# lmxyy/sige

Hardware: AMD Instinct MI355X
Metric: DDPM-256 U-Net sparse (SIGE) forwards/s (higher is better)
Workload: dtype f32; 1 GPU; DDPM 256x256 church U-Net (ch128, mult 1-1-2-2-4-4, 113.7M params, random init), 1.2% square edit, one edited image per GPU, hipGraph replay, NHWC activations, in-place scatter ...; batch_per_gpu=1, resolution=256, parallelism=dp1

## Files before the change

include/sige_hip.h:

```cpp
#ifndef SIGE_HIP_H
#define SIGE_HIP_H

#include <stddef.h>
#include <stdint.h>

#ifdef __cplusplus
extern "C" {
#endif

#define SIGE_HIP_VERSION 309

enum {
    SIGE_HIP_OK = 0,
    SIGE_HIP_EINVAL = -1,
    SIGE_HIP_EUNSUPPORTED = -2,
    SIGE_HIP_ELAUNCH = -3,
    SIGE_HIP_ENODEVICE = -4
};

enum { SIGE_HIP_ACT_IDENTITY = 0, SIGE_HIP_ACT_SWISH = 1,
       SIGE_HIP_ACT_RELU = 2, SIGE_HIP_ACT_LEAKY = 3 , SIGE_HIP_ACT_TANH = 4 };

enum {
    SIGE_HIP_TUNE_CONV_TILE_MT = 0,
// ... 63 lines not shown
                             const int32_t *active_indices, int N, int32_t *map, void *stream);

int sige_hip_scatter_gather_f32(const float *x, const float *y, int B, int C, int H, int W,
                                int Rx, int Sx, int bH, int bW,
                                const int32_t *active_indices, int N, const int32_t *scatter_map,
                                const float *scale, int scaleB, int scaleC, int scaleH, int scaleW,
                                const float *shift, int shiftB, int shiftC, int shiftH, int shiftW,
                                int activation, int activation_first, float *out, void *stream);

int sige_hip_difference_mask_u8(const float *a, const float *b, int C, int H, int W,
                                int64_t strideC, int64_t strideH, int64_t strideW, float eps,
                                uint8_t *out, void *stream);
int sige_hip_dilate_mask_u8(const uint8_t *mask, int H, int W, int dilationH, int dilationW,
                            uint8_t *out, void *stream);
int sige_hip_mask_pyramid_levels(int H, int W, int min_h, int min_w, int *hs, int *ws, int capacity);
int sige_hip_mask_pyramid_u8(const uint8_t *mask, int H, int W, int min_h, int min_w,
                             int dilationH, int dilationW, float threshold, float eps,
                             float *scratch, size_t scratch_floats, uint8_t *out, void *stream);

int sige_hip_reduce_mask_capacity(int H, int W, int strideH, int strideW, int padH, int padW);
int sige_hip_reduce_mask_i32(const uint8_t *mask, int H, int W, int bH, int bW,
                             int strideH, int strideW, int padH, int padW,
                             int32_t *indices, int capacity, int32_t *count, void *stream);

size_t sige_hip_block_conv_packed_size(int Cout, int Cin, int kH, int kW, int R, int S,
                                       int strideH, int strideW, int groups);
int sige_hip_block_conv_pack_f32(const float *w, int Cout, int Cin, int kH, int kW,
                                 float *packed, void *stream);
int sige_hip_block_conv_f32(const float *x, int T, int Cin, int R, int S,
                            const float *packed, const float *bias, int Cout, int kH, int kW,
                            int strideH, int strideW, float *out, void *stream);
int sige_hip_block_conv_direct_f32(const float *x, int T, int Cin, int R, int S,
                                   const float *w, const float *bias, int Cout, int kH, int kW,
                                   int strideH, int strideW, int dilationH, int dilationW, int groups,
                                   float *out, void *stream);
int sige_hip_spade_modulate_nhwc_f32(
        const float *x_full, const float *x_tiles, const int32_t *map_x, int Nx, int Rx, int Sx,
        const float *scale, int scaleB, int scaleC, const float *shift, int shiftB, int shiftC,
        const float *gb_tiles, const float *gb_full, const int32_t *map_g, int Ng, int Rg, int Sg,
        int B, int C, int H, int W, int bH, int bW, const int32_t *active_indices, int N,
        int leaky, float slope, float *out, void *stream);

size_t sige_hip_block_conv_packed_size_f16c(int Cout, int Cin, int kH, int kW, int R, int S,
                                            int strideH, int strideW, int groups);
int sige_hip_block_conv_pack_f16c(const float *w, int Cout, int Cin, int kH, int kW,
                                  float *packed, void *stream);
// ... 416 lines not shown
```

sige_amd/csrc/mask_pipeline.hip:

```cpp
#include "common.hpp"

namespace sige {

constexpr int kMPThreads = 1024;

__global__ void difference_mask_kernel(const float *__restrict__ a, const float *__restrict__ b, int C, long HW,
                                       long strideC, long stridePix, float eps, uint8_t *__restrict__ out) {
    for (long p = (long)blockIdx.x * blockDim.x + threadIdx.x; p < HW; p += (long)gridDim.x * blockDim.x) {
        bool any = false;
        for (int c = 0; c < C; ++c) {
            const long o = c * strideC + p * stridePix;
            any |= fabsf(a[o] - b[o]) > eps;
        }
        out[p] = any ? 1 : 0;
    }
}

__device__ __forceinline__ uint8_t dilated(const uint8_t *__restrict__ m, int W, int h, int w, int dH, int dW, int lo, int hi) {
    if (m[(size_t)h * W + w]) return 1;
    for (int i = 1; i <= dH; ++i) {
        if (h - i >= lo && m[(size_t)(h - i) * W + w]) return 1;
        if (h + i < hi && m[(size_t)(h + i) * W + w]) return 1;
    }
    for (int i = 1; i <= dW; ++i) {
// ... 57 lines not shown
        for (long p = tid; p < n2; p += kMPThreads) {
            const int i = (int)(p / w2), j = (int)(p % w2);
            float fy = sy * ((float)i + 0.5f) - 0.5f;
            if (fy < 0.f) fy = 0.f;
            const int y0 = (int)fy, y1 = y0 + (y0 < h - 1 ? 1 : 0);
            const float ly = fy - (float)y0, hy = 1.f - ly;
            float fx = sx * ((float)j + 0.5f) - 0.5f;
            if (fx < 0.f) fx = 0.f;
            const int x0 = (int)fx, x1 = x0 + (x0 < w - 1 ? 1 : 0);
            const float lx = fx - (float)x0, hx = 1.f - lx;
            auto at = [&](int y, int x) -> float {
                const size_t q = (size_t)y * w + x;
                return cur ? cur[q] : (mask[q] ? 1.0f : 0.0f);
            };
            nxt[p] = hy * (hx * at(y0, x0) + lx * at(y0, x1)) + ly * (hx * at(y1, x0) + lx * at(y1, x1));
        }
        __syncthreads();
        cur = nxt;
        nxt = (nxt == level_a) ? level_b : level_a;
        h = h2; w = w2;
    }
}

}

using namespace sige;

extern "C" int sige_hip_difference_mask_u8(const float *a, const float *b, int C, int H, int W,
                                           int64_t strideC, int64_t strideH, int64_t strideW, float eps,
                                           uint8_t *out, void *stream) {
    SIGE_PLAN_HOOK(sige_hip_difference_mask_u8, a, b, C, H, W, strideC, strideH, strideW, eps, out, stream);
    if (C <= 0 || H <= 0 || W <= 0) return SIGE_HIP_EINVAL;
    if (!a || !b || !out) return SIGE_HIP_EINVAL;
    if (strideH != (int64_t)W * strideW) return SIGE_HIP_EUNSUPPORTED;
    const long HW = (long)H * W;
    const int blocks = (int)((HW + 255) / 256 < 2048 ? (HW + 255) / 256 : 2048);
    difference_mask_kernel<<<blocks, 256, 0, as_stream(stream)>>>(a, b, C, HW, strideC, strideW, eps, out);
    return launch_status();
}

extern "C" int sige_hip_dilate_mask_u8(const uint8_t *mask, int H, int W, int dilationH, int dilationW,
                                       uint8_t *out, void *stream) {
    SIGE_PLAN_HOOK(sige_hip_dilate_mask_u8, mask, H, W, dilationH, dilationW, out, stream);
    if (H <= 0 || W <= 0 || dilationH < 0 || dilationW < 0) return SIGE_HIP_EINVAL;
    if (!mask || !out || mask == out) return SIGE_HIP_EINVAL;
    const long n = (long)H * W;
    const int blocks = (int)((n + 255) / 256 < 2048 ? (n + 255) / 256 : 2048);
    const int sh = stacked_shift(H);
    if (sh < 0) return SIGE_HIP_EUNSUPPORTED;
// ... 38 lines not shown
```

sige_amd/hip.py:

```python
import ctypes
import os
import threading
from typing import Optional, Tuple

import torch

_PKG = os.path.dirname(os.path.abspath(__file__))
LIB_PATH = os.environ.get("SIGE_HIP_LIB", os.path.join(_PKG, "lib", "libsige_hip.so"))

ACT = {"identity": 0, "swish": 1}
ACT_EXT = {"identity": 0, "relu": 2, "leaky": 3, "tanh": 4}

_c_int, _c_vp, _c_sz = ctypes.c_int, ctypes.c_void_p, ctypes.c_size_t
_lib = None

_BC = [_c_vp, _c_int, _c_int, _c_int, _c_int]

_SIGNATURES = {
    "sige_hip_version": (_c_int, []),
    "sige_hip_error_string": (ctypes.c_char_p, [_c_int]),
    "sige_hip_device_arch": (ctypes.c_char_p, []),
    "sige_hip_launch_count": (ctypes.c_int64, []),
    "sige_hip_last_launch_device": (_c_int, []),
    "sige_hip_preload": (_c_int, []),
    "sige_hip_gather_f32": (_c_int, [_c_vp] + [_c_int] * 6 + [_c_vp, _c_int] + _BC + _BC + [_c_int, _c_int, _c_vp, _c_vp]),
    "sige_hip_scatter_f32": (_c_int, [_c_vp, _c_vp] + [_c_int] * 10 + [_c_vp, _c_int] + _BC + [_c_vp, _c_vp]),
    "sige_hip_scatter_with_block_residual_f32": (
        _c_int, [_c_vp] * 4 + [_c_int] * 12 + [_c_vp, _c_int, _c_vp, _c_int, _c_vp, _c_vp]),
    "sige_hip_tile_table_i32": (_c_int, [_c_vp] + [_c_int] * 9 + [_c_vp, _c_vp]),
    "sige_hip_scatter_fused_f32": (_c_int, [_c_vp, _c_vp] + [_c_int] * 6 + [_c_vp, _c_int, _c_int, _c_int] + _BC + [_c_vp, _c_vp]),
    "sige_hip_scatter_with_block_residual_fused_f32": (
        _c_int, [_c_vp] * 4 + [_c_int] * 8 + [_c_vp, _c_int, _c_int, _c_int] * 2 + [_c_vp, _c_vp]),
    "sige_hip_scatter_map_i32": (_c_int, [_c_int] * 10 + [_c_vp, _c_int, _c_vp, _c_vp]),
    "sige_hip_scatter_gather_f32": (
        _c_int, [_c_vp, _c_vp] + [_c_int] * 8 + [_c_vp, _c_int, _c_vp] + _BC + _BC + [_c_int, _c_int, _c_vp, _c_vp]),
    "sige_hip_difference_mask_u8": (_c_int, [_c_vp, _c_vp] + [_c_int] * 3 + [ctypes.c_int64] * 3 + [ctypes.c_float, _c_vp, _c_vp]),
    "sige_hip_dilate_mask_u8": (_c_int, [_c_vp] + [_c_int] * 4 + [_c_vp, _c_vp]),
    "sige_hip_mask_pyramid_levels": (_c_int, [_c_int] * 4 + [_c_vp, _c_vp, _c_int]),
    "sige_hip_mask_pyramid_u8": (_c_int, [_c_vp] + [_c_int] * 6 + [ctypes.c_float] * 2 + [_c_vp, _c_sz, _c_vp, _c_vp]),
    "sige_hip_reduce_mask_capacity": (_c_int, [_c_int] * 6),
    "sige_hip_reduce_mask_i32": (_c_int, [_c_vp] + [_c_int] * 8 + [_c_vp, _c_int, _c_vp, _c_vp]),
    "sige_hip_block_conv_packed_size": (_c_sz, [_c_int] * 9),
    "sige_hip_block_conv_packed_size_f16c": (_c_sz, [_c_int] * 9),
    "sige_hip_block_conv_pack_f16c": (_c_int, [_c_vp] + [_c_int] * 4 + [_c_vp, _c_vp]),
    "sige_hip_block_conv_pack_f32": (_c_int, [_c_vp] + [_c_int] * 4 + [_c_vp, _c_vp]),
    "sige_hip_block_conv_f32": (_c_int, [_c_vp] + [_c_int] * 4 + [_c_vp, _c_vp] + [_c_int] * 5 + [_c_vp, _c_vp]),
    "sige_hip_gather_conv_f32": (
        _c_int, [_c_vp] + [_c_int] * 6 + [_c_vp, _c_int] + _BC + _BC + [_c_int, _c_vp, _c_vp] + [_c_int] * 5 + [_c_vp, _c_vp]),
    "sige_hip_scatter_gather_conv_f32": (
        _c_int, [_c_vp, _c_vp] + [_c_int] * 8 + [_c_vp, _c_int, _c_vp] + _BC + _BC + [_c_int, _c_vp, _c_vp]
        + [_c_int] * 5 + [_c_vp, _c_vp]),
    "sige_hip_gather_conv_nchw_f32": (
        _c_int, [_c_vp, _c_vp] + [_c_int] * 7 + [_c_vp, _c_int] + [_c_vp, _c_int, _c_int] * 2 + [_c_int, _c_vp, _c_vp]
        + [_c_int] * 7 + [_c_vp, _c_int, _c_int, _c_vp, _c_vp]),
    "sige_hip_group_norm_affine_workspace": (_c_sz, [_c_int] * 5),
    "sige_hip_group_norm_affine_f32": (_c_int, [_c_vp] + [_c_int] * 5 + [ctypes.c_float] + [_c_vp] * 6),
    "sige_hip_block_conv_direct_f32": (_c_int, [_c_vp] + [_c_int] * 4 + [_c_vp, _c_vp] + [_c_int] * 8 + [_c_vp, _c_vp]),
    "sige_hip_conv_pair_begin": (_c_int, []),
    "sige_hip_conv_pair_end": (_c_int, []),
    "sige_hip_conv_pairs_fused": (ctypes.c_int64, []),
    "sige_hip_attention_workspace": (_c_sz, [_c_int] * 3),
    "sige_hip_attention_f32": (_c_int, [_c_vp, _c_int, _c_int, _c_int, ctypes.c_float, _c_vp, _c_vp, _c_vp]),
    "sige_hip_copy_f32": (_c_int, [_c_vp, _c_vp, _c_sz, _c_vp]),
    "sige_hip_block_conv_nhwc_f32": (_c_int, [_c_vp] + [_c_int] * 4 + [_c_vp, _c_vp] + [_c_int] * 5 + [_c_vp, _c_vp]),
# ... 517 lines not shown
        table1.data_ptr(), table1.shape[0], table1.shape[1], n1, out.data_ptr(), _stream(y0)),
        "scatter_with_block_residual_fused")
    return out


def reduce_mask(mask: torch.Tensor, block_size, stride, padding) -> torch.Tensor:
    if mask.dim() != 2 or not mask.is_cuda:
        raise RuntimeError("sige_amd.hip.reduce_mask: expected a 2-D CUDA mask")
    if plan_recorder() is not None:
        return reduce_mask_batch([(mask, block_size, stride, padding)])[0]
    m = mask if mask.dtype in (torch.bool, torch.uint8) else (mask != 0)
    m = m.contiguous()
    H, W = m.shape
    cap = lib().sige_hip_reduce_mask_capacity(H, W, stride[0], stride[1], padding[0], padding[1])
    buf = torch.empty((cap + 1, 2), dtype=torch.int32, device=m.device)
    count = buf[cap]
    _check(lib().sige_hip_reduce_mask_i32(m.data_ptr(), H, W, block_size[0], block_size[1], stride[0], stride[1],
                                          padding[0], padding[1], buf.data_ptr(), cap, count.data_ptr(),
                                          _stream(m)), "reduce_mask")
    n = int(count[0].item())
    return buf[:n].clone()


def reduce_mask_batch(requests) -> list:
    if not requests:
        return []
    dev = requests[0][0].device
    counts = torch.empty(len(requests), dtype=torch.int32, device=dev)
    bufs = []
    for i, (mask, block, stride, padding) in enumerate(requests):
        if mask.dim() != 2 or not mask.is_cuda or mask.device != dev:
            raise RuntimeError("sige_amd.hip.reduce_mask_batch: expected 2-D masks on one GPU")
        m = mask if mask.dtype in (torch.bool, torch.uint8) else (mask != 0)
        m = m.contiguous()
        H, W = m.shape
        cap = lib().sige_hip_reduce_mask_capacity(H, W, stride[0], stride[1], padding[0], padding[1])
        buf = torch.empty((max(cap, 1), 2), dtype=torch.int32, device=dev)
        _check(lib().sige_hip_reduce_mask_i32(m.data_ptr(), H, W, block[0], block[1], stride[0], stride[1],
                                              padding[0], padding[1], buf.data_ptr(), cap,
                                              counts.data_ptr() + 4 * i, _stream(m)), "reduce_mask")
        bufs.append((buf, m))
    rec = plan_recorder()
    if rec is not None:
        first = rec.new_slots(len(requests))
        _check(lib().sige_hip_plan_record_readback(rec.handle, counts.data_ptr(), first, len(requests)), "plan_record_readback")
        ns = counts.cpu().tolist()
        out = []
        for i, ((buf, m), n) in enumerate(zip(bufs, ns)):
            rec.bind_index_list(buf, first + i, n)
            rec.keep.extend((buf, m))
            out.append(buf[:n])
        rec.keep.append(counts)
        return out
    ns = counts.cpu().tolist()
    return [buf[:n].clone() for (buf, _), n in zip(bufs, ns)]


def difference_mask(tensor1: torch.Tensor, tensor2: torch.Tensor, eps: float) -> torch.Tensor:
    if tensor1.shape != tensor2.shape:
        raise RuntimeError("difference_mask: shapes differ")
    a, b = tensor1, tensor2
    if a.dim() == 4:
        assert a.shape[0] == 1
        a, b = a[0], b[0]
    if a.dim() == 2:
        a, b = a[None], b[None]
    if a.dim() != 3:
        raise NotImplementedError("Unknown mask dimension [%d]!!!" % tensor1.dim())
    if not (a.is_cuda and b.is_cuda and a.dtype == b.dtype == torch.float32):
        raise NotImplementedError("difference_mask: fp32 GPU tensors")
    if a.stride() != b.stride() or a.stride(1) != a.shape[2] * a.stride(2):
        a, b = a.contiguous(), b.contiguous()
    C, H, W = a.shape
    out = torch.empty((H, W), dtype=torch.uint8, device=a.device)
    _check(lib().sige_hip_difference_mask_u8(a.data_ptr(), b.data_ptr(), C, H, W, a.stride(0), a.stride(1), a.stride(2),
                                             float(eps), out.data_ptr(), _stream(a)), "difference_mask")
    return out.view(torch.bool)

# ... 1289 lines not shown
```

sige_amd/nn/base.py:

```python
from typing import Dict, List, Optional, Tuple

import torch
from torch import nn
from torch.nn import functional as F

from .. import runtime as _runtime
from . import deferred

MODES = ("full", "sparse", "profile")


class _RuntimeTable(dict):

    def __init__(self, function_name: str):
        super().__init__()
        self.function_name = function_name

    def __missing__(self, device_type: str):
        fn = _runtime.resolve(device_type, self.function_name)
        if fn is not None:
            self[device_type] = fn
        return fn


# ... 183 lines not shown

    def _sige_modules(self):
        return (m for m in self.modules() if isinstance(m, SIGEModule))

    def set_masks(self, masks: Dict[Tuple[int, int], torch.Tensor]):
        self.timestamp += 1
        cache = {}
        self._prebuild_indices(masks, cache)
        for module in self._sige_modules():
            module.set_mask(masks, cache, self.timestamp)

    def _prebuild_indices(self, masks, cache):
        from .gather import Gather

        keys, reqs = [], []
        for m in self._sige_modules():
            if isinstance(m, Gather) and m.input_res is not None and not m.verbose:
                res = tuple(m.input_res)
                mask = masks.get(res)
                key = m.index_key(res)
                if mask is not None and mask.is_cuda and mask.dim() == 2 and key not in cache and key not in keys:
                    keys.append(key)
                    reqs.append((mask, m.block_size, m.block_stride, m.offset))
        if reqs:
            from .. import hip

            for key, idx in zip(keys, hip.reduce_mask_batch(reqs)):
                cache[key] = idx

    def set_mode(self, mode: str):
        self.mode = mode
        for module in self._sige_modules():
            module.set_mode(mode)

    def clear_cache(self):
        for module in self._sige_modules():
            module.clear_cache()

    def set_cache_id(self, cache_id: int):
        for module in self._sige_modules():
            module.set_cache_id(cache_id)

    def set_sparse_update(self, sparse_update: bool):
        for module in self._sige_modules():
            module.set_sparse_update(sparse_update)

    def set_compute_dtype(self, dtype: str, keep=None, edit_ratio: Optional[float] = None):
        if dtype not in ("f32", "f16", "f16x3"):
            raise ValueError("compute dtype must be 'f32', 'f16' or 'f16x3'")
        if keep is None:
            keep = ()
# ... 35 lines not shown
```

sige_amd/nn/dense.py:

```python
from typing import Optional, Tuple

import torch
from torch import nn
from torch.nn import functional as F

_GEOMETRY = {
    ((3, 3), (1, 1), (1, 1)): ((6, 6), (4, 4), (1, 1)),
    ((1, 1), (1, 1), (0, 0)): ((4, 4), (4, 4), (0, 0)),
    ((3, 3), (2, 2), (0, 0)): ((5, 5), (2, 2), (0, 0)),
}


def _tile_compute(compute: str) -> str:
    return compute if compute in ("f16", "f16x3") else "f32"


WIDE_MIN_FLOP = {3: 4.0e9, 1: 2.0e9}
WIDE_MIN_FLOP_X3 = {3: 4.0e9, 1: 2.0e9}
WIDE_MIN_FLOP_FULL_PASS = {3: 0.25e9, 1: 2.0e9}
WIDE_MIN_FLOP_F32 = {3: 1.0e30, 1: 1.0e30}
WIDE_MIN_FLOP_F32_STACKED = {3: 8.0e9, 1: 1.0e30}
FULL_PASS_F32_NATIVE = False
TILE_X3_MIN_FLOP = 2.0e9

# ... 109 lines not shown
    if getattr(conv, "_sige_plain_key", None) != key:
        conv._sige_plain = w.detach().contiguous()
        conv._sige_plain_key = key
    return conv._sige_plain


def fusable(conv: nn.Conv2d) -> bool:
    geo = (tuple(conv.kernel_size), tuple(conv.stride), tuple(conv.padding))
    return geo in _GEOMETRY and conv.groups == 1 and tuple(conv.dilation) == (1, 1)


def _act(x, name):
    if name == "swish":
        return F.silu(x)
    if name == "identity":
        return x
    raise ValueError("Unknown activation: [%s]!!!" % name)


def fused_conv2d(conv: nn.Conv2d, x: torch.Tensor, scale: Optional[torch.Tensor] = None,
                 shift: Optional[torch.Tensor] = None, activation_name: str = "identity",
                 x2: Optional[torch.Tensor] = None, residual: Optional[torch.Tensor] = None,
                 pad_bottom_right: bool = False, out_affine: Optional[tuple] = None,
                 twins: Optional[dict] = None) -> torch.Tensor:
    made = {}
    out = _fused_conv2d(conv, x, scale, shift, activation_name, x2, residual, pad_bottom_right, out_affine, twins, made)
    if isinstance(out, tuple):
        out, (os_, oh_, oact) = out
        out = _act(out * os_.reshape(1, -1, 1, 1) + oh_.reshape(1, -1, 1, 1), oact)
    if not made and twins and out_affine is None:
        from . import scatter

        if scatter.EMULATE_TWINS:
            made = scatter.emulated_twins(out, twins)
    out._sige_twins = made
    return out


def _fused_conv2d(conv, x, scale, shift, activation_name, x2, residual, pad_bottom_right, out_affine, twins=None, made=None):
    if x.is_cuda and x.dtype == torch.float32 and fusable(conv):
        from .. import hip

        block, out_tile, offset = _GEOMETRY[(tuple(conv.kernel_size), tuple(conv.stride), tuple(conv.padding))]
        if not pad_bottom_right:
            out = _wide_conv(conv, x, x2, scale, shift, activation_name, residual, out_affine, twins, made)
            if out is not None:
                return out
        if x2 is not None and not hip.cat_fusable(x.shape[0], x.shape[1], conv.kernel_size):
            x, x2 = torch.cat([x, x2], dim=1), None
        B, _, H, W = x.shape
        if conv.stride[0] == 2:
            if not pad_bottom_right:
                raise NotImplementedError("stride-2 fused conv expects the (0,1,0,1) padding of the DDPM downsample")
            Ho, Wo = (H + 1 - 3) // 2 + 1, (W + 1 - 3) // 2 + 1
        else:
            Ho, Wo = H, W
        if (hip.is_cl(x) and conv.out_channels <= 4 and tuple(conv.kernel_size) == (3, 3) and conv.stride[0] == 1
                and x2 is None and residual is None and out_affine is None):
            out = hip.conv3x3_small_cout_cl(x, _plain_weight(conv), conv.bias, scale, shift, activation_name)
            if out is not None:
                return out
        idx = hip.all_tiles(H, W, out_tile, conv.stride, offset, x.device)
        if hip.is_cl(x) and hip.cl_supported(x.shape[1], 0 if x2 is None else x2.shape[1], conv.out_channels):
            tw = []
            if twins and out_affine is None:
                for key, (sc, sh) in list(twins.items())[:2]:
# ... 85 lines not shown
```

sige_amd/plan.py:

```python
import ctypes
from typing import Callable, Dict, Optional

import torch

from . import hip
from .graphs import GraphPool
from .nn.base import SIGEModel
from .nn.gather import Gather

MASKS, FORWARD = 0, 1


class _Recorder:

    def __init__(self, plan: "LaunchPlan", section: int):
        self.plan = plan
        self.handle = plan.handle
        self.section = section
        self.keep = plan._keep
        self.idx_info = plan._idx_info

    def new_slots(self, n: int) -> int:
        first = hip.lib().sige_hip_plan_new_slots(self.handle, n)
        if first < 0:
# ... 136 lines not shown
        self.mask.copy_(mask, non_blocking=True)
        self._run(MASKS)
        self._read_counts()
        if bound and self.counts != self._recorded_counts:
            self.mask.copy_(prev, non_blocking=True)
            self._run(MASKS)
            self._read_counts()
            raise RuntimeError("LaunchPlan: this plan recorded calls whose sizes cannot follow a new mask (NCHW or unfused tile "
                               "kernels, or %d count argument(s) on index lists the plan does not own); it only replays masks "
                               "with the recorded tile counts -- the previous mask is still bound" % self.unbound_counts)
        self.graph = None
        if adopt:
            self._adopt()

    def _adopt(self):
        views = {}
        for ptr, (slot, cap, buf) in self._idx_info.items():
            views[ptr] = buf[:self.counts[slot]]
        for m in self.model.modules():
            if isinstance(m, Gather) and m.active_indices is not None:
                v = views.get(hip.base_ptr(m.active_indices))
                if v is not None:
                    m.active_indices = v

    def run(self) -> torch.Tensor:
        self._run(FORWARD)
        return self.out

    def capture(self):
        if self.pool is None:
            raise RuntimeError("LaunchPlan.capture before record")
        self.graph = None
        self.graph, _ = self.pool.capture(lambda: self.run())
        return self.graph

    def replay(self) -> torch.Tensor:
        if self.graph is None:
            self.capture()
        self.graph.replay()
        return self.out
```

sige_amd/utils.py:

```python
from typing import Dict, Optional, Tuple, Union

import numpy as np
import torch
from torch.nn import functional as F

IntPair = Union[int, Tuple[int, int]]


def _pair(v: IntPair) -> Tuple[int, int]:
    return (v, v) if isinstance(v, int) else (int(v[0]), int(v[1]))


def reduce_mask(
    mask: torch.Tensor,
    block_size: Optional[IntPair],
    stride: Optional[IntPair],
    padding: Optional[IntPair],
    verbose: bool = False,
) -> Optional[torch.Tensor]:
    if block_size is None or stride is None or padding is None:
        return None
    block_size, stride, padding = _pair(block_size), _pair(stride), _pair(padding)
    if mask.is_cuda:
        from . import hip
# ... 73 lines not shown
    mask: torch.Tensor,
    min_res: IntPair = 4,
    dilation: IntPair = 1,
    threshold: float = 0.3,
    eps: float = 1e-3,
) -> Dict[Tuple[int, int], torch.Tensor]:
    assert mask.dim() == 2
    H, W = mask.shape
    min_h, min_w = _pair(min_res)
    if mask.is_cuda and mask.dtype == torch.bool:
        from . import hip

        return hip.mask_pyramid(mask, (min_h, min_w), _pair(dilation), threshold, eps)
    level = mask.reshape(1, 1, H, W).float()
    h, w = H, W
    pyramid = {}
    while True:
        t = min(threshold, level.max() - eps)
        pyramid[(h, w)] = dilate_mask(level[0, 0] > t, dilation)
        h, w = h // 2, w // 2
        if h < min_h and w < min_w:
            return pyramid
        level = F.interpolate(level, (h, w), mode="bilinear", align_corners=False)
```

sige_amd/workloads/ddpm_unet.py:

```python
import math
from dataclasses import dataclass
from typing import Optional, Tuple

import torch
from torch import nn
from torch.nn import functional as F

from ..nn import Gather, Scatter, ScatterGather, ScatterWithBlockResidual, SIGEConv2d, SIGEModel, SIGEModule, paired_convs
from ..nn.deferred import lazy_cat
from ..nn.dense import fast_full_pass, full_conv2d, fused_conv2d, group_norm_affine, input_conv2d


@dataclass
class DDPMConfig:
    ch: int = 128
    ch_mult: Tuple[int, ...] = (1, 1, 2, 2, 4, 4)
    num_res_blocks: int = 2
    attn_resolutions: Tuple[int, ...] = (16,)
    in_ch: int = 3
    out_ch: int = 3
    resolution: int = 256
    main_block: Optional[int] = 6
    shortcut_block: Optional[int] = 4
    sparse_threshold: int = 64
    groups: int = 32
    eps: float = 1e-6
    reference_attn_quirk: bool = False
    preactivate: bool = True
    pair_shortcut: bool = True
    conv1_twins: bool = True
    overlap_shortcut: bool = False


# ... 179 lines not shown
                    self.scatter_gather.cache_activated(s2, t2)
                    self.scatter_gather.cache_id = keep

    def _shortcut_async(self, fn, x_ready: torch.Tensor):
        if not (self.overlap and x_ready.is_cuda and self.mode == "sparse"):
            return fn(), (lambda: None)
        cur = torch.cuda.current_stream(x_ready.device)
        if self._side is None:
            self._side = torch.cuda.Stream(device=x_ready.device)
        side = self._side
        side.wait_stream(cur)
        with torch.cuda.stream(side):
            out = fn()

        def join():
            cur.wait_stream(side)
            out.record_stream(cur)

        return out, join

    def _pairing(self, t: torch.Tensor):
        return paired_convs(t, enabled=self.pair and self.cin != self.cout and self.mode == "sparse")

    def forward(self, x, temb: Optional[torch.Tensor]) -> torch.Tensor:
        pair = x if isinstance(x, (tuple, list)) else None
        if self.mode == "full":
            if pair and not self.plain and self._fast_full() and pair[0].is_cuda:
                return self._full(pair[0], temb, x2=pair[1])
            return self._full(torch.cat(pair, dim=1) if pair else x, temb)
        if self.mode in ("sparse", "profile"):
            if pair and not self.sparse_main and self.mode == "sparse":
                return self._sparse_dense(pair[0], pair[1])
            if pair and self.mode == "sparse" and self.cin != self.cout:
                return self._sparse(lazy_cat(pair[0], pair[1]))
            return self._sparse(torch.cat(pair, dim=1) if pair else x)
        raise NotImplementedError("Unknown mode [%s]!!!" % self.mode)

    def _fast_full(self) -> bool:
        from ..nn import dense as _dense

        return _dense.fast_full_pass(self.conv1)

    def _shortcut(self, x, x2=None):
        if self.cin == self.cout:
            return x if x2 is None else torch.cat([x, x2], dim=1)
        if x2 is not None:
            if self.sparse_shortcut:
                self.shortcut_gather.note_full_input(x.shape[2:])
            return full_conv2d(self.nin_shortcut, x, x2=x2)
        if self.sparse_shortcut:
            x = self.shortcut_gather(x)
        return full_conv2d(self.nin_shortcut, x) if self.mode == "full" else self.nin_shortcut(x)

    def _plain(self, x, temb):
        skip = x if self.cin == self.cout else self.nin_shortcut(x)
# ... 40 lines not shown
        if self.sparse_main and self.preactivate and self.mode == "sparse":
            parts = list(x.parts) if hasattr(x, "parts") else [x]
            first = parts[0]
            tw = self._twin_inputs(parts, s1, t1)
            with self._pairing(first):
                skip, join = (self._shortcut_async(lambda: self._shortcut(x), first) if self.cin != self.cout
                              else (x, lambda: None))
                if tw is not None:
                    xa = tw[0] if len(tw) == 1 else lazy_cat(tw[0], tw[1])
                    h = self.conv1(self.main_gather(xa, preactivated=True), out_affine=(s2, t2, "swish"))
                else:
                    h = self.conv1(self.main_gather(x, s1, t1), out_affine=(s2, t2, "swish"))
            tiles = self.scatter_gather(h, preactivated=True)
            join()
            return self._produced(self.scatter.forward_fused(self.conv2, tiles, skip))
        if not self.sparse_main:
            return self._sparse_dense(x, None)
        skip = self._shortcut(x)
        h = self.conv1(self.main_gather(x, s1, t1))
        if self.mode == "sparse":
            return self.scatter.forward_fused(self.conv2, self.scatter_gather(h, s2, t2), skip)
        return self.scatter(self.conv2(self.scatter_gather(h, s2, t2)), skip)

    def _sparse_dense(self, x, x2):
        s1, t1, s2, t2 = self.affine[self.cache_id]
        join = lambda: None
        if self.preactivate:
            tw = self._twin_inputs([x] if x2 is None else [x, x2], s1, t1)
            with self._pairing(x):
                if self.cin == self.cout:
                    skip = x if x2 is None else torch.cat([x, x2], dim=1)
                else:
                    skip, join = self._shortcut_async(lambda: fused_conv2d(self.nin_shortcut, x, x2=x2), x)
                if tw is not None:
                    h = fused_conv2d(self.conv1, tw[0], None, None, "identity", x2=(tw[1] if len(tw) > 1 else None),
                                     out_affine=(s2, t2, "swish"))
                else:
                    h = fused_conv2d(self.conv1, x, s1, t1, "swish", x2=x2, out_affine=(s2, t2, "swish"))
            join()
            return self._produced(fused_conv2d(self.conv2, h, residual=skip, twins=self._my_twins()))
        if self.cin == self.cout:
            skip = x if x2 is None else torch.cat([x, x2], dim=1)
        else:
            skip, join = self._shortcut_async(lambda: fused_conv2d(self.nin_shortcut, x, x2=x2), x)
        join()
        h = fused_conv2d(self.conv1, x, s1, t1, "swish", x2=x2)
        return fused_conv2d(self.conv2, h, s2, t2, "swish", residual=skip)


class AttnBlock(SIGEModule, _TwinProducer):
    def __init__(self, cfg: DDPMConfig, ch: int, sparse: bool):
        super().__init__()
        self.ch = ch
        self.edit_batch = 1
        self.twin_regs = {}
        self.quirk = cfg.reference_attn_quirk
        self.sparse = sparse and cfg.shortcut_block is not None
        Conv = SIGEConv2d if self.sparse else nn.Conv2d
        self.norm = nn.GroupNorm(cfg.groups, ch, eps=cfg.eps)
        self.qkv = Conv(ch, 3 * ch, 1, 1, 0)
        self.proj_out = Conv(ch, ch, 1, 1, 0)
        if self.sparse:
            self.gather1 = Gather(self.qkv, cfg.shortcut_block)
# ... 308 lines not shown
        e = F.silu(self.temb.dense[0](e))
        e = F.silu(self.temb.dense[1](e))
        return list(torch.split(self.temb.dense[2](e), self.temb_slices, dim=1))

    SPARSE_CONV_IN = True

    def _conv_in(self, x, native_full):
        if self.mode != "sparse" and not native_full:
            return self.conv_in(x)
        if self.mode == "sparse" and self.SPARSE_CONV_IN and self.edit_batch == 1 and x.is_cuda:
            first, last = self.down[0].block[0], self.up[0].block[-1]
            g0, g1 = getattr(first, "main_gather", None), getattr(last, "main_gather", None)
            if (g0 is not None and g1 is not None and g0.active_indices is not None and g1.active_indices is not None
                    and tuple(g0.block_size) == tuple(g1.block_size) and tuple(g0.offset) == tuple(g1.offset)
                    and tuple(g0.model_stride) == (1, 1) and tuple(g1.model_stride) == (1, 1)
                    and g0.active_indices.data_ptr() == g1.active_indices.data_ptr()):
                buf = getattr(self, "_h0_buf", None)
                shape = (x.shape[0], self.conv_in.out_channels, x.shape[2], x.shape[3])
                if buf is None or tuple(buf.shape) != shape or buf.device != x.device:
                    buf = self._h0_buf = torch.zeros(shape, dtype=torch.float32, device=x.device).contiguous(memory_format=torch.channels_last)
                return input_conv2d(self.conv_in, x, tiles=(g0.active_indices, tuple(g0.block_size)), out=buf)
        return input_conv2d(self.conv_in, x)

    def forward(self, x: torch.Tensor, t: torch.Tensor) -> torch.Tensor:
        assert x.shape[2] == x.shape[3] == self.resolution
        temb = self._temb(t)
        nxt = (lambda: temb.pop(0)) if temb is not None else (lambda: None)

        from ..nn import dense as _dense

        native_full = self.mode == "full" and x.is_cuda and not getattr(self.conv_in, "_plain_model", False) and (
            getattr(self.conv_out, "compute_dtype", "f32") != "f32" or _dense.FULL_PASS_F32_NATIVE)
        h0 = self._conv_in(x, native_full)
        if x.is_contiguous(memory_format=torch.channels_last) and not x.is_contiguous():
            h0 = h0.contiguous(memory_format=torch.channels_last)
        E = self.edit_batch
        if E > 1:
            if self.mode != "sparse" or x.shape[0] != E:
                raise RuntimeError("stacked edits: sparse mode, one input image per edit")
            from ..stacked import tall, untall

            h0 = tall(h0)
        hs = [h0]
        for lvl, stage in enumerate(self.down):
            for i, block in enumerate(stage.block):
                h = block(hs[-1], nxt())
                if len(stage.attn):
                    h = stage.attn[i](h)
                hs.append(h)
            if lvl != self.num_levels - 1:
                hs.append(stage.downsample(hs[-1]))

        h = self.mid.block_1(hs[-1], nxt())
        h = self.mid.attn_1(h)
        h = self.mid.block_2(h, nxt())

        for lvl in reversed(range(self.num_levels)):
            stage = self.up[lvl]
            for i, block in enumerate(stage.block):
                h = block((h, hs.pop()), nxt())
                if len(stage.attn):
                    h = stage.attn[i](h)
            if lvl != 0:
                h = stage.upsample(h)
        if self.mode == "sparse" or native_full:
            if E > 1:
                h = untall(h, E)
            so, to = group_norm_affine(h, self.norm_out)
            return fused_conv2d(self.conv_out, h, so, to, "swish")
        return self.conv_out(F.silu(self.norm_out(h)))
```

Baseline: 780.4 forward/s.

## Compute dense up-stage convs only on demand tiles feeding the sparse upsample

```diff
diff --git a/include/sige_hip.h b/include/sige_hip.h
--- a/include/sige_hip.h
+++ b/include/sige_hip.h
@@ -109,6 +109,11 @@
 int sige_hip_reduce_mask_i32(const uint8_t *mask, int H, int W, int bH, int bW,
                              int strideH, int strideW, int padH, int padW,
                              int32_t *indices, int capacity, int32_t *count, void *stream);
+
+int sige_hip_demand_tiles_capacity(int Hp, int Wp, int tileH, int tileW);
+int sige_hip_demand_tiles_i32(const int32_t *indices, const int32_t *count, int capacity, int bH, int bW,
+                              int inH, int inW, int upsample2x, int Hp, int Wp, int tileH, int tileW,
+                              int padH, int padW, int depth, int32_t *lists, int32_t *counts, void *stream);
 
 size_t sige_hip_block_conv_packed_size(int Cout, int Cin, int kH, int kW, int R, int S,
                                        int strideH, int strideW, int groups);
diff --git a/sige_amd/csrc/mask_pipeline.hip b/sige_amd/csrc/mask_pipeline.hip
--- a/sige_amd/csrc/mask_pipeline.hip
+++ b/sige_amd/csrc/mask_pipeline.hip
@@ -103,9 +103,92 @@
     }
 }
 
+constexpr int kDTThreads = 1024, kDTMaxPix = 16384, kDTMaxCells = 4096;
+
+__global__ __launch_bounds__(kDTThreads) void demand_tiles_kernel(
+        const int32_t *__restrict__ idx, const int32_t *__restrict__ count, int capacity, int bH, int bW, int inH, int inW, int up,
+        int Hp, int Wp, int oH, int oW, int padH, int padW, int depth, int32_t *__restrict__ lists, int32_t *__restrict__ counts) {
+    __shared__ uint8_t s_map[2][kDTMaxPix];
+    __shared__ uint8_t s_flag[kDTMaxCells];
+    const int tid = threadIdx.x;
+    const int npix = Hp * Wp, gh = (Hp + oH - 1) / oH, gw = (Wp + oW - 1) / oW, ncell = gh * gw;
+    for (int p = tid; p < npix; p += kDTThreads) s_map[0][p] = 0;
+    __syncthreads();
+    int n = *count;
+    n = n < 0 ? 0 : (n > capacity ? capacity : n);
+    const int bpix = bH * bW;
+    for (long i = tid; i < (long)n * bpix; i += kDTThreads) {
+        const int t = (int)(i / bpix), r = (int)(i % bpix);
+        const int y = idx[2 * t] + r / bW, x = idx[2 * t + 1] + r % bW;
+        if (y < 0 || y >= inH || x < 0 || x >= inW) continue;
+        const int py = y >> up, px = x >> up;
+        if (py < Hp && px < Wp) s_map[0][py * Wp + px] = 1;
+    }
+    __syncthreads();
+    int cur = 0;
+    for (int k = 0; k < depth; ++k) {
+        const uint8_t *m = s_map[cur];
+        for (int c = tid; c < ncell; c += kDTThreads) {
+            const int y0 = (c / gw) * oH, x0 = (c % gw) * oW;
+            const int y1 = y0 + oH < Hp ? y0 + oH : Hp, x1 = x0 + oW < Wp ? x0 + oW : Wp;
+            uint8_t any = 0;
+            for (int y = y0; y < y1; ++y)
+                for (int x = x0; x < x1; ++x) any |= m[y * Wp + x];
+            s_flag[c] = any;
+        }
+        __syncthreads();
+        int32_t *main_list = lists + (size_t)k * ncell * 2, *flat_list = lists + ((size_t)depth + k) * ncell * 2;
+        for (int c = tid; c < ncell; c += kDTThreads) {
+            if (!s_flag[c] && c != ncell - 1) continue;
+            int rank = 0;
+            for (int j = 0; j < c; ++j) rank += s_flag[j];
+            if (s_flag[c]) {
+                const int y0 = (c / gw) * oH, x0 = (c % gw) * oW;
+                main_list[2 * rank] = y0 - padH; main_list[2 * rank + 1] = x0 - padW;
+                flat_list[2 * rank] = y0; flat_list[2 * rank + 1] = x0;
+            }
+            if (c == ncell - 1) counts[k] = rank + s_flag[c];
+        }
+        if (k + 1 < depth) {
+            uint8_t *d = s_map[cur ^ 1];
+            for (int p = tid; p < npix; p += kDTThreads) {
+                const int y = p / Wp, x = p % Wp;
+                uint8_t any = 0;
+                for (int yy = (y > 0 ? y - 1 : 0); yy <= (y + 1 < Hp ? y + 1 : Hp - 1); ++yy)
+                    for (int xx = (x > 0 ? x - 1 : 0); xx <= (x + 1 < Wp ? x + 1 : Wp - 1); ++xx) any |= m[yy * Wp + xx];
+                d[p] = any;
+            }
+        }
+        __syncthreads();
+        cur ^= 1;
+    }
+}
+
 }
 
 using namespace sige;
+
+extern "C" int sige_hip_demand_tiles_capacity(int Hp, int Wp, int tileH, int tileW) {
+    if (Hp <= 0 || Wp <= 0 || tileH <= 0 || tileW <= 0) return SIGE_HIP_EINVAL;
+    return ((Hp + tileH - 1) / tileH) * ((Wp + tileW - 1) / tileW);
+}
+
+extern "C" int sige_hip_demand_tiles_i32(const int32_t *indices, const int32_t *count, int capacity, int bH, int bW,
+                                         int inH, int inW, int upsample2x, int Hp, int Wp, int tileH, int tileW,
+                                         int padH, int padW, int depth, int32_t *lists, int32_t *counts, void *stream) {
+    SIGE_PLAN_HOOK(sige_hip_demand_tiles_i32, indices, count, capacity, bH, bW, inH, inW, upsample2x, Hp, Wp, tileH, tileW, padH, padW, depth, lists, counts, stream);
+    if (capacity < 0 || bH <= 0 || bW <= 0 || inH <= 0 || inW <= 0 || Hp <= 0 || Wp <= 0 || tileH <= 0 || tileW <= 0 ||
+        padH < 0 || padW < 0 || depth <= 0)
+        return SIGE_HIP_EINVAL;
+    if (!count || !lists || !counts || (capacity > 0 && !indices)) return SIGE_HIP_EINVAL;
+    const int up = upsample2x ? 1 : 0;
+    if (inH != (Hp << up) || inW != (Wp << up)) return SIGE_HIP_EINVAL;
+    if (stacked_shift(Hp) != 0) return SIGE_HIP_EUNSUPPORTED;
+    if ((long)Hp * Wp > kDTMaxPix || sige_hip_demand_tiles_capacity(Hp, Wp, tileH, tileW) > kDTMaxCells) return SIGE_HIP_EUNSUPPORTED;
+    demand_tiles_kernel<<<1, kDTThreads, 0, as_stream(stream)>>>(indices, count, capacity, bH, bW, inH, inW, up, Hp, Wp, tileH, tileW,
+                                                                padH, padW, depth, lists, counts);
+    return launch_status();
+}
 
 extern "C" int sige_hip_difference_mask_u8(const float *a, const float *b, int C, int H, int W,
                                            int64_t strideC, int64_t strideH, int64_t strideW, float eps,
diff --git a/sige_amd/hip.py b/sige_amd/hip.py
--- a/sige_amd/hip.py
+++ b/sige_amd/hip.py
@@ -40,6 +40,8 @@
     "sige_hip_mask_pyramid_u8": (_c_int, [_c_vp] + [_c_int] * 6 + [ctypes.c_float] * 2 + [_c_vp, _c_sz, _c_vp, _c_vp]),
     "sige_hip_reduce_mask_capacity": (_c_int, [_c_int] * 6),
     "sige_hip_reduce_mask_i32": (_c_int, [_c_vp] + [_c_int] * 8 + [_c_vp, _c_int, _c_vp, _c_vp]),
+    "sige_hip_demand_tiles_capacity": (_c_int, [_c_int] * 4),
+    "sige_hip_demand_tiles_i32": (_c_int, [_c_vp, _c_vp] + [_c_int] * 13 + [_c_vp, _c_vp, _c_vp]),
     "sige_hip_block_conv_packed_size": (_c_sz, [_c_int] * 9),
     "sige_hip_block_conv_packed_size_f16c": (_c_sz, [_c_int] * 9),
     "sige_hip_block_conv_pack_f16c": (_c_int, [_c_vp] + [_c_int] * 4 + [_c_vp, _c_vp]),
@@ -603,11 +605,22 @@
     return buf[:n].clone()
 
 
-def reduce_mask_batch(requests) -> list:
+class DemandTiles:
+
+    def __init__(self, main, flat, cells: int):
+        self.main, self.flat, self.cells = list(main), list(flat), int(cells)
+
+    @property
+    def counts(self):
+        return [int(t.shape[0]) for t in self.main]
+
+
+def reduce_mask_batch(requests, demands=None):
     if not requests:
-        return []
+        return [] if demands is None else ([], [])
     dev = requests[0][0].device
-    counts = torch.empty(len(requests), dtype=torch.int32, device=dev)
+    n_req = len(requests)
+    counts = torch.empty(n_req + sum(d[6] for d in demands or ()), dtype=torch.int32, device=dev)
     bufs = []
     for i, (mask, block, stride, padding) in enumerate(requests):
         if mask.dim() != 2 or not mask.is_cuda or mask.device != dev:
@@ -620,21 +633,47 @@
         _check(lib().sige_hip_reduce_mask_i32(m.data_ptr(), H, W, block[0], block[1], stride[0], stride[1],
                                               padding[0], padding[1], buf.data_ptr(), cap,
                                               counts.data_ptr() + 4 * i, _stream(m)), "reduce_mask")
-        bufs.append((buf, m))
+        bufs.append((buf, m, cap))
+    dbufs, at = [], n_req
+    for (i, in_res, up, prod_res, out_tile, pad, depth) in demands or ():
+        buf, m, cap = bufs[i]
+        block = requests[i][1]
+        cells = lib().sige_hip_demand_tiles_capacity(prod_res[0], prod_res[1], out_tile[0], out_tile[1])
+        if cells <= 0:
+            raise RuntimeError("sige_amd.hip.reduce_mask_batch: bad demand-region geometry")
+        lists = torch.empty((2, depth, cells, 2), dtype=torch.int32, device=dev)
+        _check(lib().sige_hip_demand_tiles_i32(buf.data_ptr(), counts.data_ptr() + 4 * i, cap, block[0], block[1], in_res[0], in_res[1],
+                                               int(bool(up)), prod_res[0], prod_res[1], out_tile[0], out_tile[1], pad[0], pad[1],
+                                               depth, lists.data_ptr(), counts.data_ptr() + 4 * at, _stream(m)), "demand_tiles")
+        dbufs.append((lists, at, depth, cells))
+        at += depth
     rec = plan_recorder()
     if rec is not None:
-        first = rec.new_slots(len(requests))
-        _check(lib().sige_hip_plan_record_readback(rec.handle, counts.data_ptr(), first, len(requests)), "plan_record_readback")
+        first = rec.new_slots(counts.numel())
+        _check(lib().sige_hip_plan_record_readback(rec.handle, counts.data_ptr(), first, counts.numel()), "plan_record_readback")
         ns = counts.cpu().tolist()
         out = []
-        for i, ((buf, m), n) in enumerate(zip(bufs, ns)):
+        for i, ((buf, m, _), n) in enumerate(zip(bufs, ns)):
             rec.bind_index_list(buf, first + i, n)
             rec.keep.extend((buf, m))
             out.append(buf[:n])
+        dout = []
+        for lists, at, depth, cells in dbufs:
+            for g in range(2):
+                for k in range(depth):
+                    rec.bind_index_list(lists[g, k], first + at + k, ns[at + k])
+            rec.keep.append(lists)
+            dout.append(DemandTiles([lists[0, k, :ns[at + k]] for k in range(depth)],
+                                    [lists[1, k, :ns[at + k]] for k in range(depth)], cells))
         rec.keep.append(counts)
+        return out if demands is None else (out, dout)
+    ns = counts.cpu().tolist()
+    out = [buf[:n].clone() for (buf, _, _), n in zip(bufs, ns)]
+    if demands is None:
         return out
-    ns = counts.cpu().tolist()
-    return [buf[:n].clone() for (buf, _), n in zip(bufs, ns)]
+    dout = [DemandTiles([lists[0, k, :ns[at + k]] for k in range(depth)], [lists[1, k, :ns[at + k]] for k in range(depth)], cells)
+            for lists, at, depth, cells in dbufs]
+    return out, dout
 
 
 def difference_mask(tensor1: torch.Tensor, tensor2: torch.Tensor, eps: float) -> torch.Tensor:
diff --git a/sige_amd/nn/base.py b/sige_amd/nn/base.py
--- a/sige_amd/nn/base.py
+++ b/sige_amd/nn/base.py
@@ -229,11 +229,33 @@
                 if mask is not None and mask.is_cuda and mask.dim() == 2 and key not in cache and key not in keys:
                     keys.append(key)
                     reqs.append((mask, m.block_size, m.block_stride, m.offset))
+        self._demand_lists = {}
+        demands = []
+        for name, g, up, prod_res, depth in self._demand_requests(masks):
+            key = g.index_key(tuple(g.input_res))
+            if key in keys:
+                demands.append((name, ("demand_tiles", *key[1:], int(up), *prod_res, *g.out_tile, *g.offset, depth),
+                                (keys.index(key), tuple(g.input_res), up, tuple(prod_res), tuple(g.out_tile), tuple(g.offset), depth)))
         if reqs:
             from .. import hip
 
-            for key, idx in zip(keys, hip.reduce_mask_batch(reqs)):
+            lists, regions = hip.reduce_mask_batch(reqs, [d[2] for d in demands])
+            for key, idx in zip(keys, lists):
                 cache[key] = idx
+            for (name, key, _), region in zip(demands, regions):
+                cache[key] = region
+                self._demand_lists[name] = region
+
+    def _demand_requests(self, masks):
+        return []
+
+    def adopt_index_lists(self, view_of):
+        for region in getattr(self, "_demand_lists", {}).values():
+            for lists in (region.main, region.flat):
+                for k, t in enumerate(lists):
+                    v = view_of(t)
+                    if v is not None:
+                        lists[k] = v
 
     def set_mode(self, mode: str):
         self.mode = mode
diff --git a/sige_amd/nn/dense.py b/sige_amd/nn/dense.py
--- a/sige_amd/nn/dense.py
+++ b/sige_amd/nn/dense.py
@@ -155,9 +155,11 @@
                  shift: Optional[torch.Tensor] = None, activation_name: str = "identity",
                  x2: Optional[torch.Tensor] = None, residual: Optional[torch.Tensor] = None,
                  pad_bottom_right: bool = False, out_affine: Optional[tuple] = None,
-                 twins: Optional[dict] = None) -> torch.Tensor:
+                 twins: Optional[dict] = None, tiles: Optional[torch.Tensor] = None,
+                 out: Optional[torch.Tensor] = None) -> torch.Tensor:
     made = {}
-    out = _fused_conv2d(conv, x, scale, shift, activation_name, x2, residual, pad_bottom_right, out_affine, twins, made)
+    out = _fused_conv2d(conv, x, scale, shift, activation_name, x2, residual, pad_bottom_right, out_affine, twins, made,
+                        tiles, out)
     if isinstance(out, tuple):
         out, (os_, oh_, oact) = out
         out = _act(out * os_.reshape(1, -1, 1, 1) + oh_.reshape(1, -1, 1, 1), oact)
@@ -170,11 +172,45 @@
     return out
 
 
-def _fused_conv2d(conv, x, scale, shift, activation_name, x2, residual, pad_bottom_right, out_affine, twins=None, made=None):
+def demand_buffer(conv: nn.Conv2d, name, shape, device) -> torch.Tensor:
+    bufs = conv.__dict__.setdefault("_sige_demand_bufs", {})
+    buf = bufs.get(name)
+    if buf is None or tuple(buf.shape) != tuple(shape) or buf.device != device:
+        buf = torch.zeros(tuple(shape), dtype=torch.float32, device=device).contiguous(memory_format=torch.channels_last)
+        bufs[name] = buf
+    return buf
+
+
+def _demand_twin_buffers(conv: nn.Conv2d, keys, shape, device):
+    bufs = conv.__dict__.setdefault("_sige_demand_bufs", {})
+    for name in [n for n in bufs if isinstance(n, tuple) and n[0] == "twin" and n[1] not in keys]:
+        del bufs[name]
+    return [demand_buffer(conv, ("twin", k), shape, device) for k in keys]
+
+
+def _fused_conv2d(conv, x, scale, shift, activation_name, x2, residual, pad_bottom_right, out_affine, twins=None, made=None,
+                  tiles=None, out_buf=None):
     if x.is_cuda and x.dtype == torch.float32 and fusable(conv):
         from .. import hip
 
         block, out_tile, offset = _GEOMETRY[(tuple(conv.kernel_size), tuple(conv.stride), tuple(conv.padding))]
+        partial = (tiles is not None and out_buf is not None and not pad_bottom_right and conv.stride[0] == 1 and hip.is_cl(x)
+                   and (x2 is None or (hip.is_cl(x2) and hip.cat_fusable(x.shape[0], x.shape[1], conv.kernel_size)))
+                   and hip.cl_supported(x.shape[1], 0 if x2 is None else x2.shape[1], conv.out_channels))
+        if partial:
+            B, _, H, W = x.shape
+            keys = list(twins)[:2] if twins and out_affine is None else []
+            tbufs = _demand_twin_buffers(conv, keys, (B, conv.out_channels, H, W), x.device)
+            tw = [(k, b, *twins[k]) for k, b in zip(keys, tbufs)]
+            out = hip.gather_conv_cl(x, x2, block, tiles, scale, shift, activation_name, _packed(conv, block), conv.bias,
+                                     conv.out_channels, conv.kernel_size, conv.stride,
+                                     full=dict(offset=offset, out_res=(H, W), residual=residual), out_affine=out_affine,
+                                     out=out_buf, twins=[(b, sc, sh) for _, b, sc, sh in tw] or None)
+            if out is None:
+                raise RuntimeError("fused_conv2d: no tile kernel for this conv over a partial tile list")
+            if made is not None:
+                made.update({k: b for k, b, _, _ in tw})
+            return out
         if not pad_bottom_right:
             out = _wide_conv(conv, x, x2, scale, shift, activation_name, residual, out_affine, twins, made)
             if out is not None:
diff --git a/sige_amd/plan.py b/sige_amd/plan.py
--- a/sige_amd/plan.py
+++ b/sige_amd/plan.py
@@ -182,6 +182,9 @@
                 v = views.get(hip.base_ptr(m.active_indices))
                 if v is not None:
                     m.active_indices = v
+        adopt = getattr(self.model, "adopt_index_lists", None)
+        if adopt is not None:
+            adopt(lambda t: views.get(hip.base_ptr(t)))
 
     def run(self) -> torch.Tensor:
         self._run(FORWARD)
diff --git a/sige_amd/utils.py b/sige_amd/utils.py
--- a/sige_amd/utils.py
+++ b/sige_amd/utils.py
@@ -119,3 +119,43 @@
         if h < min_h and w < min_w:
             return pyramid
         level = F.interpolate(level, (h, w), mode="bilinear", align_corners=False)
+
+
+def demand_tiles(
+    active_indices: torch.Tensor,
+    block_size: IntPair,
+    in_res: IntPair,
+    upsample2x: bool,
+    producer_res: IntPair,
+    out_tile: IntPair = 4,
+    padding: IntPair = 1,
+    depth: int = 1,
+):
+    (bh, bw), (ih, iw), (hp, wp) = _pair(block_size), _pair(in_res), _pair(producer_res)
+    (oh, ow), (ph, pw) = _pair(out_tile), _pair(padding)
+    up = 1 if upsample2x else 0
+    if (ih, iw) != (hp << up, wp << up):
+        raise ValueError("demand_tiles: in_res must be producer_res (times 2 with upsample2x)")
+    need = torch.zeros((hp, wp), dtype=torch.bool)
+    for y0, x0 in active_indices.cpu().tolist():
+        ys, xs = max(y0, 0), max(x0, 0)
+        ye, xe = min(y0 + bh, ih), min(x0 + bw, iw)
+        if ys < ye and xs < xe:
+            need[ys >> up:((ye - 1) >> up) + 1, xs >> up:((xe - 1) >> up) + 1] = True
+    gh, gw = -(-hp // oh), -(-wp // ow)
+    main, flat = [], []
+    for k in range(depth):
+        padded = torch.zeros((gh * oh, gw * ow), dtype=torch.bool)
+        padded[:hp, :wp] = need
+        cells = torch.nonzero(padded.reshape(gh, oh, gw, ow).any(dim=3).any(dim=1))
+        origin = torch.stack((cells[:, 0] * oh, cells[:, 1] * ow), dim=1).to(torch.int32)
+        flat.append(origin.contiguous())
+        main.append((origin - torch.tensor([ph, pw], dtype=torch.int32)).contiguous())
+        if k + 1 < depth:
+            grown = need.clone()
+            for dy in (-1, 0, 1):
+                for dx in (-1, 0, 1):
+                    src = need[max(-dy, 0):hp - max(dy, 0), max(-dx, 0):wp - max(dx, 0)]
+                    grown[max(dy, 0):hp - max(-dy, 0), max(dx, 0):wp - max(-dx, 0)] |= src
+            need = grown
+    return main, flat
diff --git a/sige_amd/workloads/ddpm_unet.py b/sige_amd/workloads/ddpm_unet.py
--- a/sige_amd/workloads/ddpm_unet.py
+++ b/sige_amd/workloads/ddpm_unet.py
@@ -8,7 +8,7 @@
 
 from ..nn import Gather, Scatter, ScatterGather, ScatterWithBlockResidual, SIGEConv2d, SIGEModel, SIGEModule, paired_convs
 from ..nn.deferred import lazy_cat
-from ..nn.dense import fast_full_pass, full_conv2d, fused_conv2d, group_norm_affine, input_conv2d
+from ..nn.dense import demand_buffer, fast_full_pass, full_conv2d, fused_conv2d, group_norm_affine, input_conv2d
 
 
 @dataclass
@@ -234,7 +234,7 @@
     def _pairing(self, t: torch.Tensor):
         return paired_convs(t, enabled=self.pair and self.cin != self.cout and self.mode == "sparse")
 
-    def forward(self, x, temb: Optional[torch.Tensor]) -> torch.Tensor:
+    def forward(self, x, temb: Optional[torch.Tensor], demand=None) -> torch.Tensor:
         pair = x if isinstance(x, (tuple, list)) else None
         if self.mode == "full":
             if pair and not self.plain and self._fast_full() and pair[0].is_cuda:
@@ -242,7 +242,7 @@
             return self._full(torch.cat(pair, dim=1) if pair else x, temb)
         if self.mode in ("sparse", "profile"):
             if pair and not self.sparse_main and self.mode == "sparse":
-                return self._sparse_dense(pair[0], pair[1])
+                return self._sparse_dense(pair[0], pair[1], demand)
             if pair and self.mode == "sparse" and self.cin != self.cout:
                 return self._sparse(lazy_cat(pair[0], pair[1]))
             return self._sparse(torch.cat(pair, dim=1) if pair else x)
@@ -329,7 +329,20 @@
             return self.scatter.forward_fused(self.conv2, self.scatter_gather(h, s2, t2), skip)
         return self.scatter(self.conv2(self.scatter_gather(h, s2, t2)), skip)
 
-    def _sparse_dense(self, x, x2):
+    def _demand_args(self, conv, demand, deeper: int, x) -> dict:
+        if demand is None:
+            return {}
+        from .. import hip
+
+        region, depth = demand
+        lists = region.flat if tuple(conv.kernel_size) == (1, 1) else region.main
+        tiles = lists[depth + deeper]
+        if tiles.shape[0] == region.cells and hip.plan_recorder() is None:
+            return {}
+        shape = (x.shape[0], conv.out_channels, x.shape[2], x.shape[3])
+        return dict(tiles=tiles, out=demand_buffer(conv, "out", shape, x.device))
+
+    def _sparse_dense(self, x, x2, demand=None):
         s1, t1, s2, t2 = self.affine[self.cache_id]
         join = lambda: None
         if self.preactivate:
@@ -338,14 +351,17 @@
                 if self.cin == self.cout:
                     skip = x if x2 is None else torch.cat([x, x2], dim=1)
                 else:
-                    skip, join = self._shortcut_async(lambda: fused_conv2d(self.nin_shortcut, x, x2=x2), x)
+                    skip, join = self._shortcut_async(lambda: fused_conv2d(self.nin_shortcut, x, x2=x2,
+                                                                           **self._demand_args(self.nin_shortcut, demand, 0, x)), x)
                 if tw is not None:
                     h = fused_conv2d(self.conv1, tw[0], None, None, "identity", x2=(tw[1] if len(tw) > 1 else None),
-                                     out_affine=(s2, t2, "swish"))
+                                     out_affine=(s2, t2, "swish"), **self._demand_args(self.conv1, demand, 1, x))
                 else:
-                    h = fused_conv2d(self.conv1, x, s1, t1, "swish", x2=x2, out_affine=(s2, t2, "swish"))
+                    h = fused_conv2d(self.conv1, x, s1, t1, "swish", x2=x2, out_affine=(s2, t2, "swish"),
+                                     **self._demand_args(self.conv1, demand, 1, x))
             join()
-            return self._produced(fused_conv2d(self.conv2, h, residual=skip, twins=self._my_twins()))
+            return self._produced(fused_conv2d(self.conv2, h, residual=skip, twins=self._my_twins(),
+                                               **self._demand_args(self.conv2, demand, 0, x)))
         if self.cin == self.cout:
             skip = x if x2 is None else torch.cat([x, x2], dim=1)
         else:
@@ -700,6 +716,55 @@
                 return input_conv2d(self.conv_in, x, tiles=(g0.active_indices, tuple(g0.block_size)), out=buf)
         return input_conv2d(self.conv_in, x)
 
+    DENSE_ON_DEMAND = True
+
+    def _demand_stages(self):
+        out = []
+        for lvl, stage in enumerate(self.up):
+            up = getattr(stage, "upsample", None)
+            if up is None or len(stage.attn) or up.gather.input_res is None:
+                continue
+            if any(b.sparse_main or not b.preactivate or b.overlap for b in stage.block):
+                continue
+            if min(up.gather.input_res) // 2 <= 4 * len(stage.block):
+                continue
+            out.append(("up.%d" % lvl, stage))
+        return out
+
+    def _demand_requests(self, masks):
+        if not self.DENSE_ON_DEMAND or self.edit_batch != 1:
+            return []
+        reqs = []
+        for name, stage in self._demand_stages():
+            g = stage.upsample.gather
+            res = tuple(g.input_res)
+            mask = masks.get(res)
+            if mask is None or not mask.is_cuda or mask.dim() != 2 or res[0] % 2 or res[1] % 2 or tuple(g.model_stride) != (1, 1):
+                continue
+            reqs.append((name, g, True, (res[0] // 2, res[1] // 2), 2 * len(stage.block)))
+        if reqs:
+            from .. import hip
+
+            if hip.get_edit_batch() != 1:
+                return []
+        return reqs
+
+    def _stage_demand(self, lvl: int, stage, h):
+        if not (self.DENSE_ON_DEMAND and self.mode == "sparse" and self.edit_batch == 1 and isinstance(h, torch.Tensor) and h.is_cuda):
+            return None
+        region = getattr(self, "_demand_lists", {}).get("up.%d" % lvl)
+        if region is None or h.shape[0] != 1:
+            return None
+        from .. import hip
+
+        convs = [c for b in stage.block for c in (b.conv1, b.conv2, getattr(b, "nin_shortcut", None)) if c is not None]
+        if not hip.is_cl(h) or any(getattr(c, "compute_dtype", "f32") != "f32" for c in convs):
+            return None
+        g = stage.upsample.gather
+        if not g.fuses_upsample(h) or tuple(g.input_res) != (2 * h.shape[2], 2 * h.shape[3]):
+            return None
+        return region
+
     def forward(self, x: torch.Tensor, t: torch.Tensor) -> torch.Tensor:
         assert x.shape[2] == x.shape[3] == self.resolution
         temb = self._temb(t)
@@ -735,8 +800,12 @@
 
         for lvl in reversed(range(self.num_levels)):
             stage = self.up[lvl]
+            region = self._stage_demand(lvl, stage, h)
             for i, block in enumerate(stage.block):
-                h = block((h, hs.pop()), nxt())
+                if region is not None:
+                    h = block((h, hs.pop()), nxt(), demand=(region, 2 * (len(stage.block) - 1 - i)))
+                else:
+                    h = block((h, hs.pop()), nxt())
                 if len(stage.attn):
                     h = stage.attn[i](h)
             if lvl != 0:
```

Result: faster. 817.4 forward/s, median of 6 (+4.7%).
